# mcgillmrl/prob_mbrl

Measured on AMD Instinct MI355X. Metric: particle_rollouts_per_sec, higher is better.
Workload: dtype f32 via split fp16 (fwd, 2 pieces) / bf16 (adjoint, 2 pieces) MFMA, fp32 accumulate

## Files before the change

### prob_mbrl_amd/csrc/pmbrl_reg.h

```cpp
#pragma once
#include <cstddef>
#include <type_traits>
#include <utility>
#include "pmbrl_dev.h"
#include "pmbrl_split.h"
#include "pmbrl_reg_head.h"
#include "pmbrl_reg_mm.h"

#define PR_NTHR (PR_NW * 64)
#define PR_NT 13
#define PR_KB 7
#define PM_GLOBAL_ __attribute__((address_space(1)))
typedef float f32x2 __attribute__((ext_vector_type(2)));

#define PR_RES_FLOATS (PR_NW * PR_SLOTS * PR_KB * 2 * PR_FRAG)
#define PR_XT_FLOATS (PR_KB * 2 * PR_FRAG)
#define PR_L0P_FLOATS (PR_NT * 2 * PR_FRAG)
#define PR_L0_FLOATS (PR_NT * PR_FRAG)
#define PR_HEAD_FLOATS (PR_NW * 2 * 2 * PR_FRAG)
#define PR_NET_FLOATS (PR_RES_FLOATS + PR_XT_FLOATS + PR_L0P_FLOATS + PR_HEAD_FLOATS)
#define PR_OFF_RES 0
#define PR_OFF_XT (PR_RES_FLOATS)
#define PR_OFF_L0 (PR_RES_FLOATS + PR_XT_FLOATS)
#define PR_OFF_HEAD (PR_RES_FLOATS + PR_XT_FLOATS + PR_L0P_FLOATS)
// ... 253 lines not shown
  r[2] = -1;
  r[3] = 0x00020000;
  return r;
}
__device__ __forceinline__ void pr_aload4_b8(unsigned (&d)[4], const pr_i32x4& srd, unsigned voff, int s0, int s1, int s2, int s3) {
  asm volatile("s_nop 4\n\tbuffer_load_ubyte %0, %4, %5, %6 offen\n\tbuffer_load_ubyte %1, %4, %5, %7 offen\n\t"
               "buffer_load_ubyte %2, %4, %5, %8 offen\n\tbuffer_load_ubyte %3, %4, %5, %9 offen"
               : "=&v"(d[0]), "=&v"(d[1]), "=&v"(d[2]), "=&v"(d[3])
               : "v"(voff), "s"(srd), "s"(s0), "s"(s1), "s"(s2), "s"(s3)
               : "memory");
}

#define PR_NRESF (2 * PR_SLOTS * PR_KB * 2)
#define PR_NAG 62
struct RegW {
  f32x4 a[PR_NAG];
  f32x4 v[PR_NRESF - PR_NAG];
};
__host__ __device__ constexpr int pr_widx(int net, int slot, int kb, int p) { return ((net * PR_SLOTS + slot) * PR_KB + kb) * 2 + p; }

template <int I>
__device__ __forceinline__ void pr_res_load(RegW& W, unsigned voff, const float* packed_dir, int wid) {
  typedef const PM_GLOBAL_ char* gcp;
  constexpr int net = I / (PR_SLOTS * PR_KB * 2), r = I % (PR_SLOTS * PR_KB * 2);
  gcp src = (gcp)(packed_dir + (size_t)net * PR_NET_FLOATS + PR_OFF_RES + ((size_t)wid * (PR_SLOTS * PR_KB * 2) + r) * PR_FRAG);
  if constexpr (I < PR_NAG) asm volatile("global_load_dwordx4 %0, %1, %2" : "=a"(W.a[I]) : "v"(voff), "s"(src) : "memory");
  else asm volatile("global_load_dwordx4 %0, %1, %2" : "=v"(W.v[I - PR_NAG]) : "v"(voff), "s"(src) : "memory");
}
template <int I>
__device__ __forceinline__ void pr_res_tie(RegW& W) {
  if constexpr (I < PR_NAG) asm volatile("" : "+a"(W.a[I]));
  else asm volatile("" : "+v"(W.v[I - PR_NAG]));
}
__device__ __forceinline__ void pr_load_resident(RegW& W, const float* packed_dir, int wid, int lane) {
  const unsigned voff = (unsigned)lane * 16u;
  pr_for<PR_NRESF>([&](auto ic) { pr_res_load<decltype(ic)::value>(W, voff, packed_dir, wid); });
  asm volatile("s_waitcnt vmcnt(0)" ::: "memory");
  pr_for<PR_NRESF>([&](auto ic) { pr_res_tie<decltype(ic)::value>(W); });
}

template <int NET, bool F16, bool XT>
__device__ __forceinline__ void pr_hidden_layer(const RegW& W, const float* lds, const float* xtw, int lane,
                                                f32x4 (&acc)[PR_SLOTS][2], f32x4 (&accx)[2]) {
  const float* act = lds + PR_LDS_ACT + lane * 4;
  f32x4 b[2][2];
  f32x4 xw[2][2];
  auto fetch = [&](int kb) {
    const int q = kb & 1;
    b[q][0] = *reinterpret_cast<const f32x4*>(act + (kb * 2 + 0) * PR_FRAG);
    b[q][1] = *reinterpret_cast<const f32x4*>(act + (kb * 2 + 1) * PR_FRAG);
    if constexpr (XT) {
      xw[q][0] = *reinterpret_cast<const f32x4*>(xtw + lane * 4 + (kb * 2 + 0) * PR_FRAG);
      xw[q][1] = *reinterpret_cast<const f32x4*>(xtw + lane * 4 + (kb * 2 + 1) * PR_FRAG);
    }
  };
  fetch(0);
  pr_for<PR_KB>([&](auto ic) {
    constexpr int kb = decltype(ic)::value;
    constexpr int q = kb & 1;
    if constexpr (kb + 1 < PR_KB) fetch(kb + 1);
    pr_for<PR_SLOTS>([&](auto sc) {
      constexpr int s = decltype(sc)::value;
      constexpr int I = pr_widx(NET, s, kb, 1);
      if constexpr (kb == 0) {
        if constexpr (I < PR_NAG) pr_mfma0<F16, true>(acc[s][0], W.a[I], b[q][0]);
        else pr_mfma0<F16, false>(acc[s][0], W.v[I - PR_NAG], b[q][0]);
      } else {
        if constexpr (I < PR_NAG) pr_mfma<F16, true>(acc[s][0], W.a[I], b[q][0]);
        else pr_mfma<F16, false>(acc[s][0], W.v[I - PR_NAG], b[q][0]);
      }
    });
// ... 78 lines not shown
  const f32x4 t = v * mf;
#pragma unroll
  for (int r = 0; r < 4; ++r) h[r] = fmaxf(t[r], 0.f);
  {
    unsigned x0, x1, x2, x3;
    asm("v_min_u32 %0, 1, %1" : "=v"(x0) : "v"(__float_as_uint(h[0])));
    asm("v_min_u32 %0, 1, %1" : "=v"(x1) : "v"(__float_as_uint(h[1])));
    asm("v_min_u32 %0, 1, %1" : "=v"(x2) : "v"(__float_as_uint(h[2])));
    asm("v_min_u32 %0, 1, %1" : "=v"(x3) : "v"(__float_as_uint(h[3])));
    unsigned a01, a23;
    asm("v_lshl_or_b32 %0, %1, 1, %2" : "=v"(a01) : "v"(x1), "v"(x0));
    asm("v_lshl_or_b32 %0, %1, 1, %2" : "=v"(a23) : "v"(x3), "v"(x2));
    asm("v_lshl_or_b32 %0, %1, 2, %2" : "=v"(ab) : "v"(a23), "v"(a01));
  }
  amax = max(max(amax, max(__float_as_uint(h[0]), __float_as_uint(h[1]))), max(__float_as_uint(h[2]), __float_as_uint(h[3])));
  if constexpr (F16) {
    const unsigned ha = pm_pk_f16(h[0], h[1]), hb = pm_pk_f16(h[2], h[3]);
    float l0, l1, l2, l3;
    asm("v_fma_mix_f32 %0, %1, -1.0, %2 op_sel:[0,0,0] op_sel_hi:[1,0,0]" : "=v"(l0) : "v"(ha), "v"(h[0]));
    asm("v_fma_mix_f32 %0, %1, -1.0, %2 op_sel:[1,0,0] op_sel_hi:[1,0,0]" : "=v"(l1) : "v"(ha), "v"(h[1]));
    asm("v_fma_mix_f32 %0, %1, -1.0, %2 op_sel:[0,0,0] op_sel_hi:[1,0,0]" : "=v"(l2) : "v"(hb), "v"(h[2]));
    asm("v_fma_mix_f32 %0, %1, -1.0, %2 op_sel:[1,0,0] op_sel_hi:[1,0,0]" : "=v"(l3) : "v"(hb), "v"(h[3]));
    hi = pm_u32x2{ha, hb};
    lo = pm_u32x2{pm_pk_f16(l0, l1), pm_pk_f16(l2, l3)};
  } else {
    pm_u32x2 pc[2];
    pm_split4<2, F16>(h, pc);
    hi = pc[0];
    lo = pc[1];
  }
}

template <int L0_BLOCKS>
__device__ __forceinline__ void pr_copy_net_to_lds(float* smem, int lds_l0, int lds_xt, int lds_head, const float* src, int tid) {
  constexpr int N_L0 = PR_NT * L0_BLOCKS * PR_FRAG / 4, N_XT = PR_XT_FLOATS / 4, N_HD = PR_HEAD_FLOATS / 4;
  constexpr int I_L0 = (N_L0 + PR_NTHR - 1) / PR_NTHR, I_XT = (N_XT + PR_NTHR - 1) / PR_NTHR, I_HD = (N_HD + PR_NTHR - 1) / PR_NTHR;
  f32x4 a[I_L0], b[I_XT], c[I_HD];
#pragma unroll
  for (int k = 0; k < I_L0; ++k) {
    const int i = min(tid + k * PR_NTHR, N_L0 - 1);
    a[k] = ldg4(src + PR_OFF_L0 + (L0_BLOCKS == 1 ? (i >> 6) * (2 * PR_FRAG) + (i & 63) * 4 : i * 4));
  }
#pragma unroll
  for (int k = 0; k < I_XT; ++k) b[k] = ldg4(src + PR_OFF_XT + min(tid + k * PR_NTHR, N_XT - 1) * 4);
#pragma unroll
  for (int k = 0; k < I_HD; ++k) c[k] = ldg4(src + PR_OFF_HEAD + min(tid + k * PR_NTHR, N_HD - 1) * 4);
#pragma unroll
  for (int k = 0; k < I_L0; ++k)
    if (tid + k * PR_NTHR < N_L0) *reinterpret_cast<f32x4*>(smem + lds_l0 + (tid + k * PR_NTHR) * 4) = a[k];
#pragma unroll
  for (int k = 0; k < I_XT; ++k)
    if (tid + k * PR_NTHR < N_XT) *reinterpret_cast<f32x4*>(smem + lds_xt + (tid + k * PR_NTHR) * 4) = b[k];
#pragma unroll
  for (int k = 0; k < I_HD; ++k)
    if (tid + k * PR_NTHR < N_HD) *reinterpret_cast<f32x4*>(smem + lds_head + (tid + k * PR_NTHR) * 4) = c[k];
}

template <bool PROF, int MMD = 0, bool TREE = false>
__global__ __launch_bounds__(PR_NTHR, 1) void pm_reg_fwd_kernel(const RegArgs A) {
  extern __shared__ __attribute__((aligned(16))) float smem[];
  constexpr bool F16 = true;
  constexpr int MMDc = MMD ? MMD : 2;
  typedef PM_GLOBAL_ uint8_t gu8;
  typedef PM_GLOBAL_ float gf32;
  typedef PM_GLOBAL_ char gch;
  const int tid = threadIdx.x, lane = tid & 63;
  const int wid = __builtin_amdgcn_readfirstlane(tid >> 6);
  const int wg = pr_wg(A);
  if (wg < 0) return;
  const int row = lane & 15, g = lane >> 4;
  int row0, nvalid;
  pr_rows(A, wg, row0, nvalid);
  const bool rvalid = row < nvalid;
  const int D = A.D, U = A.U, B = A.B;
  const float* packed = A.packed;

  if (PROF && wg == 0 && tid == 0) {
    A.prof[30] = (long long)__builtin_readcyclecounter();
    A.prof[28] = (long long)__builtin_amdgcn_s_memrealtime();
  }
  float c_mx[2], c_isx[2], c_sy[2], c_my[2], c_zp[2], c_zd[2], c_psc[2], c_pbi[2];
  float x[2];
  unsigned so_x[2], so_a[2];
  bool ok_x[2], ok_a[2];
#pragma unroll
  for (int s = 0; s < 2; ++s) {
    const int i = 2 * g + s;
    const bool isd = i < D, isa = i >= D && i < D + U;
    const int ja = isa ? i - D : 0, id = isd ? i : 0;
    c_mx[s] = (isd || isa) ? A.mx[i] : 0.f;
    c_isx[s] = (isd || isa) ? A.iSx[i] : 0.f;
    c_sy[s] = isd ? A.Sy[id] : 0.f;
    c_my[s] = isd ? A.my[id] : 0.f;
    c_zp[s] = (isa && rvalid) ? A.zpol[(size_t)(row0 + row) * U + ja] : 0.f;
    c_zd[s] = (isd && rvalid) ? A.zdyn[(size_t)(row0 + row) * D + id] : 0.f;
    c_psc[s] = isa ? A.pscale[ja] : 0.f;
    c_pbi[s] = isa ? A.pbias[ja] : 0.f;
    x[s] = (isd && rvalid) ? A.x0[(size_t)(row0 + row) * D + id] : 0.f;
    ok_x[s] = isd && rvalid;
    ok_a[s] = isa && rvalid;
    so_x[s] = ((unsigned)(row0 + row) * D + id) * 4u;
    so_a[s] = ((unsigned)(row0 + row) * U + ja) * 4u;
  }
  f32x4 hbp, hbd;
#pragma unroll
  for (int r = 0; r < 4; ++r) {
    const int rp = pr_head_row(0, D, U, 4 * g + r), rd = pr_head_row(1, D, U, 4 * g + r);
    hbp[r] = rp >= 0 ? (A.pol_params + A.pol.b_off[2])[rp] : 0.f;
    hbd[r] = rd >= 0 ? (A.dyn_params + A.dyn.b_off[2])[rd] : 0.f;
  }
  unsigned mbits[2][2][PR_SLOTS + 1];
#pragma unroll
  for (int n = 0; n < 2; ++n)
#pragma unroll
    for (int l = 0; l < 2; ++l) {
      const uint16_t* mrow = (n == 0 ? A.pol : A.dyn).mask[l] + (size_t)(row0 + (rvalid ? row : 0)) * PR_NT;
#pragma unroll
      for (int q = 0; q <= PR_SLOTS; ++q) mbits[n][l][q] = (unsigned)mrow[q < PR_SLOTS ? 4 * q + wid : PR_XT];
    }
  RegW W;
  pr_load_resident(W, packed, wid, lane);
  if (PROF && wg == 0 && tid == 0) A.prof[27] = (long long)__builtin_readcyclecounter();
#pragma unroll
  for (int s = 0; s < 2; ++s)
    if (ok_x[s] && wid == 0) *(gf32*)((gch*)A.states + so_x[s]) = x[s];
  pr_copy_net_to_lds<1>(smem, PR_LDS_L0(0), PR_LDS_XT(0), PR_LDS_HEAD(0), packed, tid);
  pr_copy_net_to_lds<1>(smem, PR_LDS_L0(1), PR_LDS_XT(1), PR_LDS_HEAD(1), packed + PR_NET_FLOATS, tid);
  if (PROF && wg == 0 && tid == 0) A.prof[26] = (long long)__builtin_readcyclecounter();
  for (int i = tid; i < PR_KB * 2 * PR_FRAG; i += PR_NTHR) smem[PR_LDS_ACT + i] = 0.f;
  if (tid < 16) smem[PR_LDS_FLAG + tid] = 0.f;
#pragma unroll
  for (int n = 0; n < 2; ++n)
#pragma unroll
    for (int l = 0; l < 2; ++l) {
      const RegNet& N = n == 0 ? A.pol : A.dyn;
#pragma unroll
      for (int q = 0; q <= PR_SLOTS; ++q) {
        if (q == PR_SLOTS && wid != pr_xwave(n)) continue;
        const unsigned nib = rvalid ? ((mbits[n][l][q] >> (4 * g)) & 0xFu) : 0u;
        f32x4 mf;
#pragma unroll
        for (int r = 0; r < 4; ++r) mf[r] = ((nib >> r) & 1u) ? N.inv_keep[l] : 0.f;
        float* dst = q < PR_SLOTS ? smem + PR_LDS_MF + (size_t)(((wid * 2 + n) * 2 + l) * PR_SLOTS + q) * PR_FRAG
                                  : smem + PR_LDS_MFX + (size_t)(n * 2 + l) * PR_FRAG;
        *reinterpret_cast<f32x4*>(dst + lane * 4) = mf;
      }
    }
  __syncthreads();
  if (tid < 64) reinterpret_cast<unsigned*>(smem + PR_LDS_ACT + ((PR_KB - 1) * 2 + 0) * PR_FRAG + tid * 4)[2] = 0x3c00u;
  if (tid == 0 && A.wflag && *A.wflag == A.wgen) atomicMin(A.status, 0);
  if (PROF && wg == 0 && tid == 0) A.prof[25] = (long long)__builtin_readcyclecounter();

  bool any_a[2], any_x[2];
#pragma unroll
  for (int s = 0; s < 2; ++s) {
    any_a[s] = false;
    any_x[s] = false;
    for (int gg = 0; gg < 4; ++gg) {
      const int i = 2 * gg + s;
      any_a[s] = any_a[s] || (i >= D && i < D + U);
      any_x[s] = any_x[s] || i < D;
    }
  }
  const float max_std_pol = expf(A.mls_pol), max_std_dyn = expf(A.mls_dyn);
  const int mm_gi = MMD ? wg / A.mm.parts : 0, mm_me = MMD ? wg - mm_gi * A.mm.parts : 0, mm_g0 = mm_gi * (MMD ? A.mm.M : 0);
  double mm_ref = 0.0;
  double* const mm_zh = reinterpret_cast<double*>(smem + PR_LDS_ZH);
  double* const mm_rec = reinterpret_cast<double*>(smem + PR_LDS_REC);
  if constexpr (MMD != 0) {
    if (wid == 0) mm_ref = row < MMD ? (double)A.x0[(size_t)mm_g0 * D + row] : 0.0;
    if (wid == 1) pr_mm_fwd_prep<MMDc>(A.mm, 0, mm_gi, mm_g0, row0, nvalid, mm_me, lane, mm_zh);
  }
  unsigned amax = 0u;
  const bool xw_pol = wid == pr_xwave(0), xw_dyn = wid == pr_xwave(1);
  float* const act_w = smem + PR_LDS_ACT + lane * 4;
  const float* const mf_w = smem + PR_LDS_MF + (size_t)wid * (2 * 2 * PR_SLOTS * PR_FRAG) + lane * 4;
  const float* const mfx_w = smem + PR_LDS_MFX + lane * 4;
  const unsigned lane_st = ((4u * g) * 16u + row) * 4u;
  const pr_rsrc srd = pr_make_rsrc(A.ws);
  const unsigned vo_abp = (unsigned)lane * 4u;
  int so_abp = (wg * PR_NW + wid) * 256;
  const int abp_step = A.nwg * (PR_NW * 256);

  auto first_layer = [&](auto netc, const float (&in)[2], int so_ab, int so_st) {
// ... 37 lines not shown
      constexpr int q = decltype(qc)::value;
      f32x4 h;
      unsigned ab;
      pm_u32x2 hi, lo;
      pr_tile_epilogue<F16>(acc[q], mfv[q], h, ab, amax, hi, lo);
      float* dst = act_w + (size_t)((ot >> 1) * 2) * PR_FRAG + 2 * (ot & 1);
      *reinterpret_cast<pm_u32x2*>(dst) = hi;
      *reinterpret_cast<pm_u32x2*>(dst + PR_FRAG) = lo;
      abw |= ab << (4 * q);
      if constexpr (NET == 0) {
#pragma unroll
        for (int r = 0; r < 4; ++r)
          PR_EXP_STASH(__builtin_amdgcn_raw_buffer_store_b32(__float_as_uint(h[r]), srd, lane_st + r * 64, pr_uni(so_st + ot * 1024), 0);)
      }
    };
    pr_for<PR_SLOTS>([&](auto qc) {
      constexpr int q = decltype(qc)::value;
      epi(qc, 4 * q + wid);
    });
    if (xw) epi(std::integral_constant<int, PR_SLOTS>{}, PR_XT);
    PR_EXP_STASH(__builtin_amdgcn_raw_buffer_store_b32(abw, srd, vo_abp, pr_uni(so_ab), 0);)
  };

  auto second_layer_and_head = [&](auto netc, int so_ab, int so_st, f32x4& o) {
    constexpr int NET = decltype(netc)::value;
    const bool xw = NET == 0 ? xw_pol : xw_dyn;
    f32x4 acc[PR_SLOTS][2], accx[2];
    f32x4 mfv[PR_SLOTS + 1], hwv[2][2];
    pr_for<PR_SLOTS>([&](auto qc) {
      constexpr int q = decltype(qc)::value;
      mfv[q] = *reinterpret_cast<const f32x4*>(mf_w + (size_t)((NET * 2 + 1) * PR_SLOTS + q) * PR_FRAG);
    });
    mfv[PR_SLOTS] = *reinterpret_cast<const f32x4*>(mfx_w + (size_t)(NET * 2 + 1) * PR_FRAG);
    if (xw) pr_hidden_layer<NET, F16, true>(W, smem, smem + PR_LDS_XT(NET), lane, acc, accx);
    else pr_hidden_layer<NET, F16, false>(W, smem, nullptr, lane, acc, accx);
    const float* hw = smem + PR_LDS_HEAD(NET) + (size_t)wid * (4 * PR_FRAG) + lane * 4;
#pragma unroll
    for (int blkk = 0; blkk < 2; ++blkk) {
      hwv[blkk][0] = *reinterpret_cast<const f32x4*>(hw + (blkk * 2 + 0) * PR_FRAG);
      hwv[blkk][1] = *reinterpret_cast<const f32x4*>(hw + (blkk * 2 + 1) * PR_FRAG);
    }
    pm_u32x2 hi[PR_SLOTS + 1], lo[PR_SLOTS + 1];
    hi[PR_SLOTS] = lo[PR_SLOTS] = pm_u32x2{0u, 0u};
    unsigned abw = 0u;
    auto epi = [&](auto qc, f32x4 v, int ot) {
      constexpr int q = decltype(qc)::value;
      f32x4 h;
      unsigned ab;
      pr_tile_epilogue<F16>(v, mfv[q], h, ab, amax, hi[q], lo[q]);
      abw |= ab << (4 * q);
      if constexpr (NET == 0) {
#pragma unroll
        for (int r = 0; r < 4; ++r)
          PR_EXP_STASH(__builtin_amdgcn_raw_buffer_store_b32(__float_as_uint(h[r]), srd, lane_st + r * 64, pr_uni(so_st + ot * 1024), 0);)
      }
    };
    pr_for<PR_SLOTS>([&](auto qc) {
      constexpr int q = decltype(qc)::value;
      epi(qc, pr_tile_value<F16>(acc[q]), 4 * q + wid);
    });
    if (xw) epi(std::integral_constant<int, PR_SLOTS>{}, pr_tile_value<F16>(accx), PR_XT);
    PR_EXP_STASH(__builtin_amdgcn_raw_buffer_store_b32(abw, srd, vo_abp, pr_uni(so_ab), 0);)
    f32x4 c0, c1, bh[2], bl[2];
#pragma unroll
    for (int blkk = 0; blkk < 2; ++blkk) {
      const pm_u32x2 ha = hi[2 * blkk], hb = hi[2 * blkk + 1], la = lo[2 * blkk], lb = lo[2 * blkk + 1];
// ... 111 lines not shown
      double rec[3] = {0.0, 0.0, 0.0};
      if (wid == 0) {
        float xo[2];
        const bool ok = pr_mm_fwd_chain<MMDc, TREE>(Q, t, Q.tag0 + (unsigned)(t + 1), mm_gi, mm_me, mm_gi * Q.parts, nvalid, ln, xs, mm_ref,
                                               mm_zh + (t & 1) * (16 * MMDc), xo, rec, xh, xtag,
                                               (PROF && wg <= 1) ? A.prof + (size_t)t * 32 + 8 * wg : nullptr);
        if (!ok && lane == 0) atomicMin(A.status, t);
        *reinterpret_cast<f32x2*>(smem + PR_LDS_XB + row * 8 + 2 * g) = f32x2{xo[0], xo[1]};
      }
      pr_barrier();
      if (wid == 0) {
#pragma unroll
        for (int i = 0; i < 3; ++i) mm_rec[i * 64 + ln] = rec[i];
      }
      const f32x2 xm = *reinterpret_cast<const f32x2*>(smem + PR_LDS_XB + row * 8 + 2 * g);
#pragma unroll
      for (int s = 0; s < 2; ++s) x[s] = ok_x[s] ? xm[s] : 0.f;
#pragma unroll
      for (int s = 0; s < 2; ++s)
        if (wid == 3 && ok_x[s]) *(gf32*)(b_states + so_x[s]) = x[s];
      if (PROF && wg == 0 && tid == 0) A.prof[(size_t)t * 32 + 7] = (long long)__builtin_readcyclecounter();
    }
#ifdef PR_EXP_AMAX_CODE
    if (amax > 0x477fe000u) atomicMin(A.status, -1);
#else
    if (amax > 0x477fe000u) atomicMin(A.status, t);
#endif
    so_abp += abp_step;
    so_st0 += st_step0; so_st1 += st_step; so_st2 += st_step;
    so_td += (int)x_step; so_tp += (int)a_step;
    b_states += x_step; b_actions += a_step; so_xt += (int)x_step;
    if (PROF && wg == 0 && tid == 0) A.prof[(size_t)t * 32 + 5] = (long long)__builtin_readcyclecounter();
  }
  if constexpr (MMD != 0) {
    pr_barrier();
    if (wid == 2 && A.H > 0) {
      const RegMM Q = pr_mm_load(pr_mm_args());
      pr_mm_fwd_file<MMDc>(Q, A.H - 1, mm_gi, mm_me, lane, mm_rec);
    }
  }
  if (PROF && wg == 0 && tid == 0) {
    A.prof[31] = (long long)__builtin_readcyclecounter();
    A.prof[29] = (long long)__builtin_amdgcn_s_memrealtime();
  }
}

struct RegUnpackArgs {
  int B, H, nwg;
  int mm_on, M, parts, rpw;
  const unsigned* src[2][2];
  unsigned char* dst[2][2];
};
__global__ __launch_bounds__(PR_NTHR) void pm_reg_unpack_abits_kernel(const RegUnpackArgs U) {
  const int wg = blockIdx.x, t = blockIdx.y, tid = threadIdx.x, wid = tid >> 6, lane = tid & 63;
  int row0 = wg * 16, nvalid = min(16, U.B - wg * 16);
  if (U.mm_on) {
    const int gi = wg / U.parts, me = wg - gi * U.parts;
    row0 = gi * U.M + me * U.rpw;
    nvalid = min(U.rpw, U.M - me * U.rpw);
  }
  const int rowg = row0 + (lane & 15), g = lane >> 4;
  if ((lane & 15) >= nvalid) return;
  for (int n = 0; n < 2; ++n)
    for (int l = 0; l < 2; ++l) {
      const unsigned w = U.src[n][l][((size_t)t * U.nwg + wg) * PR_NTHR + tid];
      unsigned char* d = U.dst[n][l] + ((size_t)t * U.B + rowg) * (PR_NT * 4) + g;
// ... 22 lines not shown
__global__ __launch_bounds__(PR_NTHR, 1) void pm_reg_bwd_kernel(const RegArgs A) {
  extern __shared__ __attribute__((aligned(16))) float smem[];
  constexpr bool F16 = false;
  constexpr int MMDc = MMD ? MMD : 2;
  typedef PM_GLOBAL_ float gf32;
  const int tid = threadIdx.x, lane = tid & 63;
  const int wid = __builtin_amdgcn_readfirstlane(tid >> 6);
  const int wg = pr_wg(A);
  if (wg < 0) return;
  const int row = lane & 15, g = lane >> 4;
  int row0, nvalid;
  pr_rows(A, wg, row0, nvalid);
  const bool rvalid = row < nvalid;
  const int D = A.D, U = A.U, B = A.B;
  const int T0 = A.t0;
  int T1 = A.t1;
  if (A.nvalid) T1 = min(T1, __builtin_amdgcn_readfirstlane(*A.nvalid));
  const float* packed = A.packed + (size_t)2 * PR_NET_FLOATS;
  if (T1 <= T0) {
    for (int i = tid; i < nvalid * D; i += PR_NTHR) {
      if (A.grad_x0 && T0 == 0) A.grad_x0[(size_t)row0 * D + i] = 0.f;
      if (A.gx_out) A.gx_out[(size_t)row0 * D + i] = A.gx_in ? A.gx_in[(size_t)row0 * D + i] : 0.f;
    }
    return;
  }

  if (PROF && wg == 0 && tid == 0) {
    A.prof[30] = (long long)__builtin_readcyclecounter();
    A.prof[28] = (long long)__builtin_amdgcn_s_memrealtime();
  }
  float c_isx[2], c_sy[2], c_psc[2], c_pbi[2];
  bool ok_x[2], ok_a[2];
  unsigned so_x[2], so_a[2];
  float gx[2] = {0.f, 0.f};
#pragma unroll
  for (int s = 0; s < 2; ++s) {
    const int i = 2 * g + s;
    const bool isd = i < D, isa = i >= D && i < D + U;
    const int ja = isa ? i - D : 0, id = isd ? i : 0;
    c_isx[s] = (isd || isa) ? A.iSx[i] : 0.f;
    c_sy[s] = isd ? A.Sy[id] : 0.f;
    c_psc[s] = isa ? A.pscale[ja] : 1.f;
    c_pbi[s] = isa ? A.pbias[ja] : 0.f;
    ok_x[s] = isd && rvalid;
    ok_a[s] = isa && rvalid;
    so_x[s] = ((unsigned)(row0 + row) * D + id) * 4u;
    so_a[s] = ((unsigned)(row0 + row) * U + ja) * 4u;
    if (A.gx_in && ok_x[s]) gx[s] = *(const gf32*)((const PM_GLOBAL_ char*)A.gx_in + so_x[s]);
  }
  RegW W;
  pr_load_resident(W, packed, wid, lane);
  pr_copy_net_to_lds<2>(smem, PRB_LDS_L0(0), PRB_LDS_XT(0), PRB_LDS_HEAD(0), packed, tid);
  pr_copy_net_to_lds<2>(smem, PRB_LDS_L0(1), PRB_LDS_XT(1), PRB_LDS_HEAD(1), packed + PR_NET_FLOATS, tid);
  for (int i = tid; i < PR_KB * 2 * PR_FRAG; i += PR_NTHR) smem[PRB_LDS_ACT + i] = 0.f;
  if (tid < 16) smem[PRB_LDS_XTAG + tid] = 0.f;
  if (tid < 64) {
    const int n = tid >> 5, l = (tid >> 4) & 1, nib = tid & 15;
    const float ik = (n == 0 ? A.pol : A.dyn).inv_keep[l];
    f32x4 m;
#pragma unroll
    for (int r = 0; r < 4; ++r) m[r] = ((nib >> r) & 1) ? ik : 0.f;
    *reinterpret_cast<f32x4*>(smem + PRB_LDS_LUT + tid * 4) = m;
  }
  __syncthreads();

  const bool xw_pol = wid == pr_xwave(0), xw_dyn = wid == pr_xwave(1);
  float* const act_w = smem + PRB_LDS_ACT + lane * 4;
  const float* const lut = smem + PRB_LDS_LUT;
  const unsigned lane_st = ((4u * g) * 16u + row) * 4u;
  const pr_rsrc srd = pr_make_rsrc(A.ws);
  const unsigned x_step = (unsigned)B * D * 4u, a_step = (unsigned)B * U * 4u;
  const int st_step = A.nwg * (PR_NT * 1024), st_step2 = A.nwg * 1024;
  int so_g0 = (int)A.gT[0] + ((T1 - 1) * A.nwg + wg) * (PR_NT * 1024);
  int so_g2 = (int)A.gT[2] + ((T1 - 1) * A.nwg + wg) * 1024;

  float* const stage = smem + PRB_LDS_IN;
  typedef const PM_GLOBAL_ char* gcp;
  gcp sp[2];
  unsigned sstep[2];
#pragma unroll
  for (int k = 0; k < 2; ++k) {
    const int e = tid + k * PR_NTHR, r = e >> 5, c = e & 31;
    const long long grow = row0 + r;
    gcp q = (gcp)A.ws;
    unsigned st = 0u;
    if (r < nvalid) {
      const int i = c >= 18 ? c - 18 : (c >= 10 ? c - 10 : c - 2);
      if (c == 0) {
        q = (gcp)A.grad_rewards + ((long long)(T1 - 1) * B + grow) * 4;
        st = (unsigned)B * 4u;
      } else if (c >= 2 && c < 26 && i < D && c < 18) {
        q = (gcp)A.ws + (c < 10 ? A.Jx : A.Td) + ((long long)(T1 - 1) * B + grow) * D * 4 + i * 4;
        st = x_step;
      } else if (c >= 2 && c < 26 && i >= D && i < D + U) {
        q = (c >= 18 ? (gcp)A.actions : (gcp)A.ws + (c < 10 ? A.Ja : A.Tp)) + ((long long)(T1 - 1) * B + grow) * U * 4 + (i - D) * 4;
        st = a_step;
      }
// ... 58 lines not shown
      mfv[q] = *reinterpret_cast<const f32x4*>(lut + ((NET * 2 + 1) * 16 + ((abw >> (4 * q)) & 15u)) * 4);
    });
    pr_mfma_open();
    pr_for<PR_SLOTS + 1>([&](auto qc) {
      constexpr int q = decltype(qc)::value;
      pr_mfma0<F16, false, true>(acc[q], wf[q][0], bf[0]);
    });
    pr_for<PR_SLOTS + 1>([&](auto qc) {
      constexpr int q = decltype(qc)::value;
      pr_mfma<F16, false, true>(acc[q], wf[q][1], bf[1]);
    });
    asm volatile("s_nop 7\n\ts_nop 7" : "+v"(acc[0]), "+v"(acc[1]), "+v"(acc[2]), "+v"(acc[3]));
    auto epi = [&](auto qc, int ot) {
      constexpr int q = decltype(qc)::value;
      const f32x4 gq = acc[q] * mfv[q];
      pm_u32x2 pc[2];
      pm_split4<2, false>(gq, pc);
      float* dst = act_w + (size_t)((ot >> 1) * 2) * PR_FRAG + 2 * (ot & 1);
      *reinterpret_cast<pm_u32x2*>(dst) = pc[0];
      *reinterpret_cast<pm_u32x2*>(dst + PR_FRAG) = pc[1];
    };
    pr_for<PR_SLOTS>([&](auto qc) {
      constexpr int q = decltype(qc)::value;
      epi(qc, 4 * q + wid);
    });
    if (xw) epi(std::integral_constant<int, PR_SLOTS>{}, PR_XT);
  };

  auto hidden_adjoint_and_tail = [&](auto netc, const unsigned abw, int so_st, f32x4& o, auto arrived) {
    constexpr int NET = decltype(netc)::value;
    const bool xw = NET == 0 ? xw_pol : xw_dyn;
    f32x4 acc[PR_SLOTS][2], accx[2];
    f32x4 mfv[PR_SLOTS + 1], hwv[2][2];
    if (xw) pr_hidden_layer<NET, F16, true>(W, smem, smem + PRB_LDS_XT(NET), lane, acc, accx);
    else pr_hidden_layer<NET, F16, false>(W, smem, nullptr, lane, acc, accx);
    arrived();
    pr_for<PR_SLOTS + 1>([&](auto qc) {
      constexpr int q = decltype(qc)::value;
      mfv[q] = *reinterpret_cast<const f32x4*>(lut + ((NET * 2 + 0) * 16 + ((abw >> (4 * q)) & 15u)) * 4);
    });
    const float* hw = smem + PRB_LDS_HEAD(NET) + (size_t)wid * (4 * PR_FRAG) + lane * 4;
#pragma unroll
    for (int blkk = 0; blkk < 2; ++blkk) {
      hwv[blkk][0] = *reinterpret_cast<const f32x4*>(hw + (blkk * 2 + 0) * PR_FRAG);
      hwv[blkk][1] = *reinterpret_cast<const f32x4*>(hw + (blkk * 2 + 1) * PR_FRAG);
    }
    pm_u32x2 hi[PR_SLOTS + 1], lo[PR_SLOTS + 1];
    hi[PR_SLOTS] = lo[PR_SLOTS] = pm_u32x2{0u, 0u};
    auto epi = [&](auto qc, f32x4 v, int ot) {
      constexpr int q = decltype(qc)::value;
      const f32x4 gq = v * mfv[q];
      pm_u32x2 pc[2];
      pm_split4<2, false>(gq, pc);
      hi[q] = pc[0];
      lo[q] = pc[1];
      if constexpr (NET == 0) {
#pragma unroll
        for (int r = 0; r < 4; ++r)
          PR_EXP_STASH(__builtin_amdgcn_raw_buffer_store_b32(__float_as_uint(gq[r]), srd, lane_st + r * 64, pr_uni(so_st + ot * 1024), 0);)
      }
    };
    pr_for<PR_SLOTS>([&](auto qc) {
      constexpr int q = decltype(qc)::value;
      epi(qc, pr_tile_value<F16>(acc[q]), 4 * q + wid);
    });
    if (xw) epi(std::integral_constant<int, PR_SLOTS>{}, pr_tile_value<F16>(accx), PR_XT);
    f32x4 c0, c1, bh[2], bl[2];
#pragma unroll
    for (int blkk = 0; blkk < 2; ++blkk) {
      const pm_u32x2 ha = hi[2 * blkk], hb = hi[2 * blkk + 1], la = lo[2 * blkk], lb = lo[2 * blkk + 1];
      bh[blkk] = __builtin_bit_cast(f32x4, (pr_u32x4){ha[0], ha[1], hb[0], hb[1]});
      bl[blkk] = __builtin_bit_cast(f32x4, (pr_u32x4){la[0], la[1], lb[0], lb[1]});
    }
    pr_mfma_open();
    pr_mfma0<F16, false, true>(c0, hwv[0][1], bh[0]);
    pr_mfma0<F16, false, true>(c1, hwv[0][0], bl[0]);
    pr_mfma<F16, false, true>(c0, hwv[1][1], bh[1]);
    pr_mfma<F16, false, true>(c1, hwv[0][0], bh[0]);
    pr_mfma<F16, false, true>(c1, hwv[1][0], bl[1]);
    pr_mfma<F16, false, true>(c1, hwv[1][0], bh[1]);
    asm volatile("s_nop 7\n\ts_nop 7" : "+v"(c0), "+v"(c1));
    float* part = smem + PRB_LDS_PART + lane * 4;
    *reinterpret_cast<f32x4*>(part + wid * PR_FRAG) = c0 + c1;
    pr_barrier();
    o = *reinterpret_cast<const f32x4*>(part);
#pragma unroll
    for (int w = 1; w < PR_NW; ++w) o += *reinterpret_cast<const f32x4*>(part + w * PR_FRAG);
  };

  const int mm_gi = MMD ? wg / A.mm.parts : 0, mm_me = MMD ? wg - mm_gi * A.mm.parts : 0, mm_g0 = mm_gi * (MMD ? A.mm.M : 0);
  double* const mm_bop = reinterpret_cast<double*>(smem + PRB_LDS_MMB);
  double* const mm_yop = reinterpret_cast<double*>(smem + PRB_LDS_MMY);
  if constexpr (MMD != 0) {
    if (wid == 1) pr_mm_bwd_prep_noise<MMDc>(A.mm, T1 - 1, mm_gi, mm_g0, row0, nvalid, lane, mm_bop + ((T1 - 1) & 1) * PR_MM_BOP_DOUBLES);
    if (wid == 2) pr_mm_bwd_prep_factor<MMDc>(A.mm, B, T1 - 1, mm_gi, row0, nvalid, lane, mm_yop + ((T1 - 1) & 1) * PR_MM_YOP_DOUBLES(MMDc));
  }
  unsigned abc[4], abn[4];
  stage_load();
  ab_load(abc);
  stage_landed(std::integral_constant<int, 0>{}, sv);
  ab_landed(std::integral_constant<int, 0>{}, abc);
  stage_park();
  __syncthreads();
  for (int t = T1 - 1; t >= T0; --t) {
    if (PROF && wg == 0 && tid == 0) A.prof[(size_t)t * 32 + 0] = (long long)__builtin_readcyclecounter();
    StepIn In;
    read_in(In);
    if constexpr (MMD != 0) {
      const bool do_chain = t < T1 - 1 || A.gx_in;
      int ln = lane;
      asm volatile("" : "+v"(ln));
      pr_mm_kptr Qp = pr_mm_args();
      asm volatile("" : "+s"(Qp));
      const RegMM Q = pr_mm_load(Qp);
      if (PROF && wg == 0 && tid == 0) A.prof[(size_t)t * 32 + 6] = (long long)__builtin_readcyclecounter();
      if (wid == 1 && t > T0) {
        pr_mm_bwd_prep_noise<MMDc>(Q, t - 1, mm_gi, mm_g0, row0, nvalid, ln, mm_bop + ((t - 1) & 1) * PR_MM_BOP_DOUBLES);
        if (PROF && wg == 0 && lane == 0) A.prof[(size_t)t * 32 + 13] = (long long)__builtin_readcyclecounter();
      } else if (wid == 2 && t > T0) {
        pr_mm_bwd_prep_factor<MMDc>(Q, B, t - 1, mm_gi, row0, nvalid, ln, mm_yop + ((t - 1) & 1) * PR_MM_YOP_DOUBLES(MMDc));
        if (PROF && wg == 0 && lane == 0) A.prof[(size_t)t * 32 + 14] = (long long)__builtin_readcyclecounter();
      }
      if (do_chain) {
        double* const xh = reinterpret_cast<double*>(smem + PRB_LDS_XH);
        volatile unsigned* const xtag = reinterpret_cast<volatile unsigned*>(smem + PRB_LDS_XTAG);
        if constexpr (TREE) {
          if (wid != 0) {
            const bool okh = pm_xch_tree_help<PR_MM_NVX(MMDc), 4>(Q.xch, Q.nwg, mm_gi * Q.parts, Q.parts, Q.fan, mm_me, Q.tag0 + (unsigned)(T1 - t), wid, xh,
                                                    xtag, ln);
            if (!okh && lane == 0 && A.status) atomicMax(A.status, 1);
          }
        }
        if (wid == 0) {
          float go[(MMDc + 3) / 4];
          const bool ok = pr_mm_bwd_chain<MMDc, TREE>(Q, Q.tag0 + (unsigned)(T1 - t), mm_me, mm_gi * Q.parts, nvalid, ln, gx,
                                                 mm_bop + (t & 1) * PR_MM_BOP_DOUBLES, mm_yop + (t & 1) * PR_MM_YOP_DOUBLES(MMDc), go,
// ... 108 lines not shown
```

Measured before the change: 6.432 million.

## Overlap kernel prologue loads and defer second-net resident weight wait into first step

Prologue loads (constants, masks, biases, and the net sections destined for LDS) are now issued as raw asynchronous global loads and only consumed after explicit vmcnt waits. Resident register weights are split per network: one network's weights are waited on before the loop, and the other's wait is deferred until its first hidden layer inside the time loop, with counted vmcnt values. The aim is to hide kernel startup memory latency behind LDS initialization and the first layer's compute. The cost is fragile hand-counted vmcnt numbers, for example 27 and 6. If these do not match the outstanding loads, the code can read weights before they arrive.

```diff
diff --git a/prob_mbrl_amd/csrc/pmbrl_reg.h b/prob_mbrl_amd/csrc/pmbrl_reg.h
--- a/prob_mbrl_amd/csrc/pmbrl_reg.h
+++ b/prob_mbrl_amd/csrc/pmbrl_reg.h
@@ -309,11 +309,38 @@
   if constexpr (I < PR_NAG) asm volatile("" : "+a"(W.a[I]));
   else asm volatile("" : "+v"(W.v[I - PR_NAG]));
 }
-__device__ __forceinline__ void pr_load_resident(RegW& W, const float* packed_dir, int wid, int lane) {
+#define PR_NRESH (PR_NRESF / 2)
+#ifdef PR_EXP_NOSTASH
+#define PR_FWD_DEFER_N 0
+#else
+#define PR_FWD_DEFER_N 27
+#endif
+#define PR_BWD_DEFER_N 6
+template <int NET>
+__device__ __forceinline__ void pr_res_issue_net(RegW& W, const float* packed_dir, int wid, int lane) {
   const unsigned voff = (unsigned)lane * 16u;
-  pr_for<PR_NRESF>([&](auto ic) { pr_res_load<decltype(ic)::value>(W, voff, packed_dir, wid); });
-  asm volatile("s_waitcnt vmcnt(0)" ::: "memory");
-  pr_for<PR_NRESF>([&](auto ic) { pr_res_tie<decltype(ic)::value>(W); });
+  pr_for<PR_NRESH>([&](auto ic) { pr_res_load<decltype(ic)::value + NET * PR_NRESH>(W, voff, packed_dir, wid); });
+}
+template <int N>
+__device__ __forceinline__ void pr_res_wait() {
+  asm volatile("s_waitcnt vmcnt(%0)" ::"n"(N) : "memory");
+}
+template <int NET>
+__device__ __forceinline__ void pr_res_tie_net(RegW& W) {
+  pr_for<PR_NRESH>([&](auto ic) { pr_res_tie<decltype(ic)::value + NET * PR_NRESH>(W); });
+}
+__device__ __forceinline__ void pr_aload_f32(float& d, const float* p) {
+  asm volatile("global_load_dword %0, %1, off" : "=v"(d) : "v"((const PM_GLOBAL_ float*)p) : "memory");
+}
+__device__ __forceinline__ void pr_aload_i32(int& d, const int* p) {
+  asm volatile("global_load_dword %0, %1, off" : "=v"(d) : "v"((const PM_GLOBAL_ int*)p) : "memory");
+}
+__device__ __forceinline__ void pr_aload_u16(unsigned& d, const uint16_t* p) {
+  asm volatile("global_load_ushort %0, %1, off" : "=v"(d) : "v"((const PM_GLOBAL_ uint16_t*)p) : "memory");
+}
+template <class T>
+__device__ __forceinline__ void pr_atie(T& d) {
+  asm volatile("" : "+v"(d));
 }
 
 template <int NET, bool F16, bool XT>
@@ -458,28 +485,46 @@
 }
 
 template <int L0_BLOCKS>
-__device__ __forceinline__ void pr_copy_net_to_lds(float* smem, int lds_l0, int lds_xt, int lds_head, const float* src, int tid) {
-  constexpr int N_L0 = PR_NT * L0_BLOCKS * PR_FRAG / 4, N_XT = PR_XT_FLOATS / 4, N_HD = PR_HEAD_FLOATS / 4;
-  constexpr int I_L0 = (N_L0 + PR_NTHR - 1) / PR_NTHR, I_XT = (N_XT + PR_NTHR - 1) / PR_NTHR, I_HD = (N_HD + PR_NTHR - 1) / PR_NTHR;
+struct RegSect {
+  static constexpr int N_L0 = PR_NT * L0_BLOCKS * PR_FRAG / 4, N_XT = PR_XT_FLOATS / 4, N_HD = PR_HEAD_FLOATS / 4;
+  static constexpr int I_L0 = (N_L0 + PR_NTHR - 1) / PR_NTHR, I_XT = (N_XT + PR_NTHR - 1) / PR_NTHR, I_HD = (N_HD + PR_NTHR - 1) / PR_NTHR;
+  static constexpr int LOADS = I_L0 + I_XT + I_HD;
   f32x4 a[I_L0], b[I_XT], c[I_HD];
-#pragma unroll
-  for (int k = 0; k < I_L0; ++k) {
-    const int i = min(tid + k * PR_NTHR, N_L0 - 1);
-    a[k] = ldg4(src + PR_OFF_L0 + (L0_BLOCKS == 1 ? (i >> 6) * (2 * PR_FRAG) + (i & 63) * 4 : i * 4));
-  }
-#pragma unroll
-  for (int k = 0; k < I_XT; ++k) b[k] = ldg4(src + PR_OFF_XT + min(tid + k * PR_NTHR, N_XT - 1) * 4);
-#pragma unroll
-  for (int k = 0; k < I_HD; ++k) c[k] = ldg4(src + PR_OFF_HEAD + min(tid + k * PR_NTHR, N_HD - 1) * 4);
-#pragma unroll
-  for (int k = 0; k < I_L0; ++k)
-    if (tid + k * PR_NTHR < N_L0) *reinterpret_cast<f32x4*>(smem + lds_l0 + (tid + k * PR_NTHR) * 4) = a[k];
-#pragma unroll
-  for (int k = 0; k < I_XT; ++k)
-    if (tid + k * PR_NTHR < N_XT) *reinterpret_cast<f32x4*>(smem + lds_xt + (tid + k * PR_NTHR) * 4) = b[k];
-#pragma unroll
-  for (int k = 0; k < I_HD; ++k)
-    if (tid + k * PR_NTHR < N_HD) *reinterpret_cast<f32x4*>(smem + lds_head + (tid + k * PR_NTHR) * 4) = c[k];
+};
+__device__ __forceinline__ void pr_sect_ld(f32x4& d, const float* base, int float_off) {
+  asm volatile("global_load_dwordx4 %0, %1, %2" : "=v"(d) : "v"((unsigned)float_off * 4u), "s"((const PM_GLOBAL_ char*)base) : "memory");
+}
+template <int L0_BLOCKS>
+__device__ __forceinline__ void pr_sect_load(RegSect<L0_BLOCKS>& S, const float* src, int tid) {
+  typedef RegSect<L0_BLOCKS> R;
+#pragma unroll
+  for (int k = 0; k < R::I_L0; ++k) {
+    const int i = min(tid + k * PR_NTHR, R::N_L0 - 1);
+    pr_sect_ld(S.a[k], src, PR_OFF_L0 + (L0_BLOCKS == 1 ? (i >> 6) * (2 * PR_FRAG) + (i & 63) * 4 : i * 4));
+  }
+#pragma unroll
+  for (int k = 0; k < R::I_XT; ++k) pr_sect_ld(S.b[k], src, PR_OFF_XT + min(tid + k * PR_NTHR, R::N_XT - 1) * 4);
+#pragma unroll
+  for (int k = 0; k < R::I_HD; ++k) pr_sect_ld(S.c[k], src, PR_OFF_HEAD + min(tid + k * PR_NTHR, R::N_HD - 1) * 4);
+}
+template <int L0_BLOCKS>
+__device__ __forceinline__ void pr_sect_store(float* smem, int lds_l0, int lds_xt, int lds_head, RegSect<L0_BLOCKS>& S, int tid) {
+  typedef RegSect<L0_BLOCKS> R;
+#pragma unroll
+  for (int k = 0; k < R::I_L0; ++k) pr_atie(S.a[k]);
+#pragma unroll
+  for (int k = 0; k < R::I_XT; ++k) pr_atie(S.b[k]);
+#pragma unroll
+  for (int k = 0; k < R::I_HD; ++k) pr_atie(S.c[k]);
+#pragma unroll
+  for (int k = 0; k < R::I_L0; ++k)
+    if (tid + k * PR_NTHR < R::N_L0) *reinterpret_cast<f32x4*>(smem + lds_l0 + (tid + k * PR_NTHR) * 4) = S.a[k];
+#pragma unroll
+  for (int k = 0; k < R::I_XT; ++k)
+    if (tid + k * PR_NTHR < R::N_XT) *reinterpret_cast<f32x4*>(smem + lds_xt + (tid + k * PR_NTHR) * 4) = S.b[k];
+#pragma unroll
+  for (int k = 0; k < R::I_HD; ++k)
+    if (tid + k * PR_NTHR < R::N_HD) *reinterpret_cast<f32x4*>(smem + lds_head + (tid + k * PR_NTHR) * 4) = S.c[k];
 }
 
 template <bool PROF, int MMD = 0, bool TREE = false>
@@ -509,52 +554,81 @@
   float x[2];
   unsigned so_x[2], so_a[2];
   bool ok_x[2], ok_a[2];
+  const int rowc = row0 + (rvalid ? row : 0);
 #pragma unroll
   for (int s = 0; s < 2; ++s) {
     const int i = 2 * g + s;
     const bool isd = i < D, isa = i >= D && i < D + U;
-    const int ja = isa ? i - D : 0, id = isd ? i : 0;
-    c_mx[s] = (isd || isa) ? A.mx[i] : 0.f;
-    c_isx[s] = (isd || isa) ? A.iSx[i] : 0.f;
-    c_sy[s] = isd ? A.Sy[id] : 0.f;
-    c_my[s] = isd ? A.my[id] : 0.f;
-    c_zp[s] = (isa && rvalid) ? A.zpol[(size_t)(row0 + row) * U + ja] : 0.f;
-    c_zd[s] = (isd && rvalid) ? A.zdyn[(size_t)(row0 + row) * D + id] : 0.f;
-    c_psc[s] = isa ? A.pscale[ja] : 0.f;
-    c_pbi[s] = isa ? A.pbias[ja] : 0.f;
-    x[s] = (isd && rvalid) ? A.x0[(size_t)(row0 + row) * D + id] : 0.f;
+    const int ja = isa ? i - D : 0, id = isd ? i : 0, ii = (isd || isa) ? i : 0;
+    pr_aload_f32(c_mx[s], A.mx + ii);
+    pr_aload_f32(c_isx[s], A.iSx + ii);
+    pr_aload_f32(c_sy[s], A.Sy + id);
+    pr_aload_f32(c_my[s], A.my + id);
+    pr_aload_f32(c_zp[s], A.zpol + (size_t)rowc * U + ja);
+    pr_aload_f32(c_zd[s], A.zdyn + (size_t)rowc * D + id);
+    pr_aload_f32(c_psc[s], A.pscale + ja);
+    pr_aload_f32(c_pbi[s], A.pbias + ja);
+    pr_aload_f32(x[s], A.x0 + (size_t)rowc * D + id);
     ok_x[s] = isd && rvalid;
     ok_a[s] = isa && rvalid;
     so_x[s] = ((unsigned)(row0 + row) * D + id) * 4u;
     so_a[s] = ((unsigned)(row0 + row) * U + ja) * 4u;
   }
   f32x4 hbp, hbd;
+  float hbp_r[4], hbd_r[4];
 #pragma unroll
   for (int r = 0; r < 4; ++r) {
     const int rp = pr_head_row(0, D, U, 4 * g + r), rd = pr_head_row(1, D, U, 4 * g + r);
-    hbp[r] = rp >= 0 ? (A.pol_params + A.pol.b_off[2])[rp] : 0.f;
-    hbd[r] = rd >= 0 ? (A.dyn_params + A.dyn.b_off[2])[rd] : 0.f;
+    pr_aload_f32(hbp_r[r], A.pol_params + A.pol.b_off[2] + (rp >= 0 ? rp : 0));
+    pr_aload_f32(hbd_r[r], A.dyn_params + A.dyn.b_off[2] + (rd >= 0 ? rd : 0));
   }
   unsigned mbits[2][2][PR_SLOTS + 1];
 #pragma unroll
   for (int n = 0; n < 2; ++n)
 #pragma unroll
     for (int l = 0; l < 2; ++l) {
-      const uint16_t* mrow = (n == 0 ? A.pol : A.dyn).mask[l] + (size_t)(row0 + (rvalid ? row : 0)) * PR_NT;
-#pragma unroll
-      for (int q = 0; q <= PR_SLOTS; ++q) mbits[n][l][q] = (unsigned)mrow[q < PR_SLOTS ? 4 * q + wid : PR_XT];
-    }
+      const uint16_t* mrow = (n == 0 ? A.pol : A.dyn).mask[l] + (size_t)rowc * PR_NT;
+#pragma unroll
+      for (int q = 0; q <= PR_SLOTS; ++q) pr_aload_u16(mbits[n][l][q], mrow + (q < PR_SLOTS ? 4 * q + wid : PR_XT));
+    }
+  int wflag_v;
+  pr_aload_i32(wflag_v, A.wflag ? A.wflag : A.status);
+  RegSect<1> S0, S1;
+  pr_sect_load(S0, packed, tid);
+  pr_sect_load(S1, packed + PR_NET_FLOATS, tid);
   RegW W;
-  pr_load_resident(W, packed, wid, lane);
+  pr_res_issue_net<0>(W, packed, wid, lane);
+#pragma unroll
+  for (int k = 0; k < PR_KB * 2 * PR_FRAG / PR_NTHR; ++k)
+    reinterpret_cast<unsigned*>(smem)[PR_LDS_ACT + tid + k * PR_NTHR] = (k == (PR_KB - 1) * 2 && (tid & 3) == 2) ? 0x3c00u : 0u;
+  if (tid < 16) smem[PR_LDS_FLAG + tid] = 0.f;
+  pr_res_wait<PR_NRESH>();
+  pr_sect_store(smem, PR_LDS_L0(0), PR_LDS_XT(0), PR_LDS_HEAD(0), S0, tid);
+  pr_sect_store(smem, PR_LDS_L0(1), PR_LDS_XT(1), PR_LDS_HEAD(1), S1, tid);
   if (PROF && wg == 0 && tid == 0) A.prof[27] = (long long)__builtin_readcyclecounter();
 #pragma unroll
-  for (int s = 0; s < 2; ++s)
-    if (ok_x[s] && wid == 0) *(gf32*)((gch*)A.states + so_x[s]) = x[s];
-  pr_copy_net_to_lds<1>(smem, PR_LDS_L0(0), PR_LDS_XT(0), PR_LDS_HEAD(0), packed, tid);
-  pr_copy_net_to_lds<1>(smem, PR_LDS_L0(1), PR_LDS_XT(1), PR_LDS_HEAD(1), packed + PR_NET_FLOATS, tid);
-  if (PROF && wg == 0 && tid == 0) A.prof[26] = (long long)__builtin_readcyclecounter();
-  for (int i = tid; i < PR_KB * 2 * PR_FRAG; i += PR_NTHR) smem[PR_LDS_ACT + i] = 0.f;
-  if (tid < 16) smem[PR_LDS_FLAG + tid] = 0.f;
+  for (int s = 0; s < 2; ++s) {
+    const int i = 2 * g + s;
+    const bool isd = i < D, isa = i >= D && i < D + U;
+    pr_atie(c_mx[s]); pr_atie(c_isx[s]); pr_atie(c_sy[s]); pr_atie(c_my[s]); pr_atie(c_zp[s]);
+    pr_atie(c_zd[s]); pr_atie(c_psc[s]); pr_atie(c_pbi[s]); pr_atie(x[s]);
+    c_mx[s] = (isd || isa) ? c_mx[s] : 0.f;
+    c_isx[s] = (isd || isa) ? c_isx[s] : 0.f;
+    c_sy[s] = isd ? c_sy[s] : 0.f;
+    c_my[s] = isd ? c_my[s] : 0.f;
+    c_zp[s] = ok_a[s] ? c_zp[s] : 0.f;
+    c_zd[s] = ok_x[s] ? c_zd[s] : 0.f;
+    c_psc[s] = isa ? c_psc[s] : 0.f;
+    c_pbi[s] = isa ? c_pbi[s] : 0.f;
+    x[s] = ok_x[s] ? x[s] : 0.f;
+  }
+#pragma unroll
+  for (int r = 0; r < 4; ++r) {
+    pr_atie(hbp_r[r]); pr_atie(hbd_r[r]);
+    hbp[r] = pr_head_row(0, D, U, 4 * g + r) >= 0 ? hbp_r[r] : 0.f;
+    hbd[r] = pr_head_row(1, D, U, 4 * g + r) >= 0 ? hbd_r[r] : 0.f;
+  }
+  pr_atie(wflag_v);
 #pragma unroll
   for (int n = 0; n < 2; ++n)
 #pragma unroll
@@ -562,6 +636,7 @@
       const RegNet& N = n == 0 ? A.pol : A.dyn;
 #pragma unroll
       for (int q = 0; q <= PR_SLOTS; ++q) {
+        pr_atie(mbits[n][l][q]);
         if (q == PR_SLOTS && wid != pr_xwave(n)) continue;
         const unsigned nib = rvalid ? ((mbits[n][l][q] >> (4 * g)) & 0xFu) : 0u;
         f32x4 mf;
@@ -572,10 +647,22 @@
         *reinterpret_cast<f32x4*>(dst + lane * 4) = mf;
       }
     }
-  __syncthreads();
-  if (tid < 64) reinterpret_cast<unsigned*>(smem + PR_LDS_ACT + ((PR_KB - 1) * 2 + 0) * PR_FRAG + tid * 4)[2] = 0x3c00u;
-  if (tid == 0 && A.wflag && *A.wflag == A.wgen) atomicMin(A.status, 0);
+  if (PROF && wg == 0 && tid == 0) A.prof[26] = (long long)__builtin_readcyclecounter();
+  pr_res_issue_net<1>(W, packed, wid, lane);
+#ifdef PR_EXP_NO_DEFER
+  pr_res_wait<0>();
+  pr_res_tie_net<0>(W);
+  pr_res_tie_net<1>(W);
+#else
+  pr_res_wait<PR_NRESH>();
+  pr_res_tie_net<0>(W);
+#endif
   if (PROF && wg == 0 && tid == 0) A.prof[25] = (long long)__builtin_readcyclecounter();
+  pr_barrier();
+#pragma unroll
+  for (int s = 0; s < 2; ++s)
+    if (ok_x[s] && wid == 0) *(gf32*)((gch*)A.states + so_x[s]) = x[s];
+  if (tid == 0 && A.wflag && wflag_v == A.wgen) atomicMin(A.status, 0);
 
   bool any_a[2], any_x[2];
 #pragma unroll
@@ -679,6 +766,12 @@
       mfv[q] = *reinterpret_cast<const f32x4*>(mf_w + (size_t)((NET * 2 + 1) * PR_SLOTS + q) * PR_FRAG);
     });
     mfv[PR_SLOTS] = *reinterpret_cast<const f32x4*>(mfx_w + (size_t)(NET * 2 + 1) * PR_FRAG);
+#ifndef PR_EXP_NO_DEFER
+    if constexpr (NET == 1) {
+      pr_res_wait<PR_FWD_DEFER_N>();
+      pr_res_tie_net<1>(W);
+    }
+#endif
     if (xw) pr_hidden_layer<NET, F16, true>(W, smem, smem + PR_LDS_XT(NET), lane, acc, accx);
     else pr_hidden_layer<NET, F16, false>(W, smem, nullptr, lane, acc, accx);
     const float* hw = smem + PR_LDS_HEAD(NET) + (size_t)wid * (4 * PR_FRAG) + lane * 4;
@@ -856,6 +949,9 @@
     b_states += x_step; b_actions += a_step; so_xt += (int)x_step;
     if (PROF && wg == 0 && tid == 0) A.prof[(size_t)t * 32 + 5] = (long long)__builtin_readcyclecounter();
   }
+#ifndef PR_EXP_NO_DEFER
+  pr_res_wait<0>();
+#endif
   if constexpr (MMD != 0) {
     pr_barrier();
     if (wid == 2 && A.H > 0) {
@@ -944,37 +1040,23 @@
   float c_isx[2], c_sy[2], c_psc[2], c_pbi[2];
   bool ok_x[2], ok_a[2];
   unsigned so_x[2], so_a[2];
-  float gx[2] = {0.f, 0.f};
+  float gx[2];
 #pragma unroll
   for (int s = 0; s < 2; ++s) {
     const int i = 2 * g + s;
     const bool isd = i < D, isa = i >= D && i < D + U;
     const int ja = isa ? i - D : 0, id = isd ? i : 0;
-    c_isx[s] = (isd || isa) ? A.iSx[i] : 0.f;
-    c_sy[s] = isd ? A.Sy[id] : 0.f;
-    c_psc[s] = isa ? A.pscale[ja] : 1.f;
-    c_pbi[s] = isa ? A.pbias[ja] : 0.f;
+    pr_aload_f32(c_isx[s], A.iSx + ((isd || isa) ? i : 0));
+    pr_aload_f32(c_sy[s], A.Sy + id);
+    pr_aload_f32(c_psc[s], A.pscale + ja);
+    pr_aload_f32(c_pbi[s], A.pbias + ja);
     ok_x[s] = isd && rvalid;
     ok_a[s] = isa && rvalid;
     so_x[s] = ((unsigned)(row0 + row) * D + id) * 4u;
     so_a[s] = ((unsigned)(row0 + row) * U + ja) * 4u;
-    if (A.gx_in && ok_x[s]) gx[s] = *(const gf32*)((const PM_GLOBAL_ char*)A.gx_in + so_x[s]);
+    pr_aload_f32(gx[s], (A.gx_in && ok_x[s]) ? A.gx_in + ((size_t)(row0 + row) * D + id) : A.Sy);
   }
   RegW W;
-  pr_load_resident(W, packed, wid, lane);
-  pr_copy_net_to_lds<2>(smem, PRB_LDS_L0(0), PRB_LDS_XT(0), PRB_LDS_HEAD(0), packed, tid);
-  pr_copy_net_to_lds<2>(smem, PRB_LDS_L0(1), PRB_LDS_XT(1), PRB_LDS_HEAD(1), packed + PR_NET_FLOATS, tid);
-  for (int i = tid; i < PR_KB * 2 * PR_FRAG; i += PR_NTHR) smem[PRB_LDS_ACT + i] = 0.f;
-  if (tid < 16) smem[PRB_LDS_XTAG + tid] = 0.f;
-  if (tid < 64) {
-    const int n = tid >> 5, l = (tid >> 4) & 1, nib = tid & 15;
-    const float ik = (n == 0 ? A.pol : A.dyn).inv_keep[l];
-    f32x4 m;
-#pragma unroll
-    for (int r = 0; r < 4; ++r) m[r] = ((nib >> r) & 1) ? ik : 0.f;
-    *reinterpret_cast<f32x4*>(smem + PRB_LDS_LUT + tid * 4) = m;
-  }
-  __syncthreads();
 
   const bool xw_pol = wid == pr_xwave(0), xw_dyn = wid == pr_xwave(1);
   float* const act_w = smem + PRB_LDS_ACT + lane * 4;
@@ -1099,6 +1181,12 @@
     const bool xw = NET == 0 ? xw_pol : xw_dyn;
     f32x4 acc[PR_SLOTS][2], accx[2];
     f32x4 mfv[PR_SLOTS + 1], hwv[2][2];
+#ifndef PR_EXP_NO_DEFER
+    if constexpr (NET == 0) {
+      pr_res_wait<PR_BWD_DEFER_N>();
+      pr_res_tie_net<0>(W);
+    }
+#endif
     if (xw) pr_hidden_layer<NET, F16, true>(W, smem, smem + PRB_LDS_XT(NET), lane, acc, accx);
     else pr_hidden_layer<NET, F16, false>(W, smem, nullptr, lane, acc, accx);
     arrived();
@@ -1158,17 +1246,56 @@
   const int mm_gi = MMD ? wg / A.mm.parts : 0, mm_me = MMD ? wg - mm_gi * A.mm.parts : 0, mm_g0 = mm_gi * (MMD ? A.mm.M : 0);
   double* const mm_bop = reinterpret_cast<double*>(smem + PRB_LDS_MMB);
   double* const mm_yop = reinterpret_cast<double*>(smem + PRB_LDS_MMY);
+  unsigned abc[4], abn[4];
+  stage_load();
+  ab_load(abc);
+  RegSect<2> S0, S1;
+  pr_sect_load(S0, packed, tid);
+  pr_sect_load(S1, packed + PR_NET_FLOATS, tid);
+  pr_res_issue_net<1>(W, packed, wid, lane);
+  for (int i = tid; i < PR_KB * 2 * PR_FRAG; i += PR_NTHR) smem[PRB_LDS_ACT + i] = 0.f;
+  if (tid < 16) smem[PRB_LDS_XTAG + tid] = 0.f;
+  if (tid < 64) {
+    const int n = tid >> 5, l = (tid >> 4) & 1, nib = tid & 15;
+    const float ik = (n == 0 ? A.pol : A.dyn).inv_keep[l];
+    f32x4 m;
+#pragma unroll
+    for (int r = 0; r < 4; ++r) m[r] = ((nib >> r) & 1) ? ik : 0.f;
+    *reinterpret_cast<f32x4*>(smem + PRB_LDS_LUT + tid * 4) = m;
+  }
+  stage_landed(std::integral_constant<int, PR_NRESH>{}, sv);
+  ab_landed(std::integral_constant<int, PR_NRESH>{}, abc);
+  pr_sect_store(smem, PRB_LDS_L0(0), PRB_LDS_XT(0), PRB_LDS_HEAD(0), S0, tid);
+  pr_sect_store(smem, PRB_LDS_L0(1), PRB_LDS_XT(1), PRB_LDS_HEAD(1), S1, tid);
+  stage_park();
+  if (PROF && wg == 0 && tid == 0) A.prof[27] = (long long)__builtin_readcyclecounter();
+#pragma unroll
+  for (int s = 0; s < 2; ++s) {
+    const int i = 2 * g + s;
+    const bool isd = i < D, isa = i >= D && i < D + U;
+    pr_atie(c_isx[s]); pr_atie(c_sy[s]); pr_atie(c_psc[s]); pr_atie(c_pbi[s]); pr_atie(gx[s]);
+    c_isx[s] = (isd || isa) ? c_isx[s] : 0.f;
+    c_sy[s] = isd ? c_sy[s] : 0.f;
+    c_psc[s] = isa ? c_psc[s] : 1.f;
+    c_pbi[s] = isa ? c_pbi[s] : 0.f;
+    gx[s] = (A.gx_in && ok_x[s]) ? gx[s] : 0.f;
+  }
+  if (PROF && wg == 0 && tid == 0) A.prof[26] = (long long)__builtin_readcyclecounter();
+  pr_res_issue_net<0>(W, packed, wid, lane);
+#ifdef PR_EXP_NO_DEFER
+  pr_res_wait<0>();
+  pr_res_tie_net<1>(W);
+  pr_res_tie_net<0>(W);
+#else
+  pr_res_wait<PR_NRESH>();
+  pr_res_tie_net<1>(W);
+#endif
+  if (PROF && wg == 0 && tid == 0) A.prof[25] = (long long)__builtin_readcyclecounter();
   if constexpr (MMD != 0) {
     if (wid == 1) pr_mm_bwd_prep_noise<MMDc>(A.mm, T1 - 1, mm_gi, mm_g0, row0, nvalid, lane, mm_bop + ((T1 - 1) & 1) * PR_MM_BOP_DOUBLES);
     if (wid == 2) pr_mm_bwd_prep_factor<MMDc>(A.mm, B, T1 - 1, mm_gi, row0, nvalid, lane, mm_yop + ((T1 - 1) & 1) * PR_MM_YOP_DOUBLES(MMDc));
   }
-  unsigned abc[4], abn[4];
-  stage_load();
-  ab_load(abc);
-  stage_landed(std::integral_constant<int, 0>{}, sv);
-  ab_landed(std::integral_constant<int, 0>{}, abc);
-  stage_park();
-  __syncthreads();
+  pr_barrier();
   for (int t = T1 - 1; t >= T0; --t) {
     if (PROF && wg == 0 && tid == 0) A.prof[(size_t)t * 32 + 0] = (long long)__builtin_readcyclecounter();
     StepIn In;
```

Measured after the change: 6.466 million, median of 6. No clear change (+0.5%).
